# IntelLabs/bayesian-torch

Hardware: AMD Instinct MI355X
Metric: MC-samples/sec (Bayesian-ResNet18, 224^2, bs=64) (higher is better)
Workload: dtype bf16

## Files before the change

bayesian_torch_amd/_lib.py:

```python
import ctypes
import os

_HERE = os.path.dirname(os.path.abspath(__file__))
_LIB = None

KIND_REPARAM, KIND_FLIPOUT = 0, 1
ACT_F32, ACT_BF16 = 0, 1
PREC_F32, PREC_BF16, PREC_BF16X3 = 0, 1, 2
PREC_CODE = {"f32": 0, "bf16": 1, "bf16x3": 2}
FLAG_TRANSPOSED, FLAG_KL_ACCUM, FLAG_ROWFUSE, FLAG_OUT_F32, FLAG_OUT_BF16, FLAG_GATHER, FLAG_SWAP_SIGNS, FLAG_CONCURRENT = 1, 2, 4, 8, 16, 32, 64, 128
FLAG_REVERSE = 256
E_UNSUPPORTED = -3
STREAM_EPS_W, STREAM_EPS_B, STREAM_SIGN_IN, STREAM_SIGN_OUT = 0, 1, 2, 3
ABI_VERSION = 9
FLAG_LANES_SHIFT = 16
FLAG_LANES_MASK = 0xff << FLAG_LANES_SHIFT
SAMPLE_SKIP_MU = 1


class BtxError(RuntimeError):
    pass


class Geom(ctypes.Structure):
    _fields_ = [(n, ctypes.c_int32) for n in (
        "NB", "D", "H", "W", "C", "N", "KD", "KH", "KW", "sd", "sh", "sw", "pd", "ph", "pw",
        "dd", "dh", "dw", "od", "oh", "ow", "groups")]


class Rng(ctypes.Structure):
    _fields_ = [("seed", ctypes.c_uint64), ("sample_idx", ctypes.c_uint32), ("layer_id", ctypes.c_uint32),
                ("sample_idx_dev", ctypes.c_void_p)]


class BnFuse(ctypes.Structure):
    _fields_ = [("residual", ctypes.c_void_p), ("relu", ctypes.c_int32), ("mask", ctypes.c_void_p), ("dres", ctypes.c_void_p)]


class Epilogue(ctypes.Structure):
    _fields_ = [("scale", ctypes.c_void_p), ("shift", ctypes.c_void_p), ("residual", ctypes.c_void_p),
                ("relu", ctypes.c_int32), ("pool", ctypes.c_int32)]


class Lanes(ctypes.Structure):
    _fields_ = [("n", ctypes.c_int32), ("x_stride", ctypes.c_int64), ("out_stride", ctypes.c_int64),
                ("res_stride", ctypes.c_int64)]


class PlanInfo(ctypes.Structure):
    _fields_ = [(n, ctypes.c_int32) for n in ("family", "ksplits", "kper", "kgroups", "wide", "tall", "par_major", "pool_band",
                                              "nwg", "lanes")] + [("ws_bytes", ctypes.c_uint64)]


FAMILIES = ("gather", "regstage", "dma", "gemm8", "patch", "taps", "taps2", "stem", "stem_pool")


class Noise(ctypes.Structure):
    _fields_ = [("eps_w", ctypes.c_void_p), ("eps_b", ctypes.c_void_p),
                ("sign_in", ctypes.c_void_p), ("sign_out", ctypes.c_void_p), ("sampled_w", ctypes.c_void_p)]


class SampleItem(ctypes.Structure):
    _fields_ = [("geom", ctypes.POINTER(Geom)), ("mu_w", ctypes.c_void_p), ("rho_w", ctypes.c_void_p),
                ("out", ctypes.c_void_p), ("kind", ctypes.c_int32), ("layer_id", ctypes.c_uint32),
                ("src_KW", ctypes.c_int32), ("src_C", ctypes.c_int32)]


class LstmLayer(ctypes.Structure):
    _fields_ = [("mu_w", ctypes.c_void_p), ("rho_w", ctypes.c_void_p), ("mu_b", ctypes.c_void_p), ("rho_b", ctypes.c_void_p),
                ("layer_id", ctypes.c_uint32), ("sample_idx", ctypes.c_uint32), ("sample_idx_dev", ctypes.c_void_p)]


class LstmGrads(ctypes.Structure):
    _fields_ = [("dmu_w", ctypes.c_void_p), ("drho_w", ctypes.c_void_p), ("dmu_b", ctypes.c_void_p), ("drho_b", ctypes.c_void_p)]


class KlItem(ctypes.Structure):
    _fields_ = [("mu", ctypes.c_void_p), ("rho", ctypes.c_void_p), ("prior_mu_t", ctypes.c_void_p),
                ("prior_sigma_t", ctypes.c_void_p), ("dmu", ctypes.c_void_p), ("drho", ctypes.c_void_p),
                ("prior_mu", ctypes.c_float), ("prior_sigma", ctypes.c_float), ("n", ctypes.c_size_t)]


class Q8Chain(ctypes.Structure):
    _fields_ = [(n, ctypes.c_float) for n in ("s_sigma", "s_mu", "s_eps", "inv_s_eps", "s_d", "inv_s_d", "inv_s_w")] + \
               [("bias_div", ctypes.c_double)]


class Q8Add(ctypes.Structure):
    _fields_ = [(n, ctypes.c_float) for n in ("s_a", "pre_a", "s_b", "pre_b", "inv_s")] + \
               [("zero_point", ctypes.c_int32), ("relu", ctypes.c_int32)]


class Q8Delta(ctypes.Structure):
    _fields_ = [("inv_s_eps", ctypes.c_float), ("mult", ctypes.c_float), ("mean_bias", ctypes.c_int32), ("pert_bias", ctypes.c_int32),
# ... 247 lines not shown
```

bayesian_torch_amd/csrc/btx_contract_taps.h:

```cpp
#pragma once
#include <type_traits>
#include "btx_contract.h"
#include "btx_contract_dma.h"
#include "btx_epilogue.h"
#include "btx_mma.h"

namespace btx {

__device__ __forceinline__ void dma16s(__amdgpu_buffer_rsrc_t rsrc, uint32_t voff, uint32_t soff,
                                       unsigned char* lds_wave_base) {
  __builtin_amdgcn_raw_ptr_buffer_load_lds(rsrc, (__attribute__((address_space(3))) void*)lds_wave_base, 16, voff, soff,
                                           0, 0);
}

template <int N>
__device__ __forceinline__ void end_stage() {
  asm volatile("s_waitcnt vmcnt(%0)\n\ts_waitcnt lgkmcnt(0)\n\ts_barrier" ::"n"(N) : "memory");
}

template <int I, int N, class F>
__device__ __forceinline__ void static_for(F&& f) {
  if constexpr (I < N) {
    f(std::integral_constant<int, I>{});
    static_for<I + 1, N>(f);
// ... 264 lines not shown
            if constexpr (t == 0) write_signs(PAR ^ 1, cb0 + cbi + 1);
          }
        }
        DeltaFrag df;
        if constexpr (KG == 1) {
          load_delta<K2>(df, smem + PT_W_OFF + wslot * DW_STAGE, l31, h);
          constexpr int t1 = (t + 1) % T, c1 = (t + 1) / T;
          load_frag(nxt, PAR ^ c1, (t1 / KW) * row_step + (t1 % KW) * p.dw, (wslot + 1) & 3, mia_tag);
          if constexpr (FIRST && t == 0) stage_mma<PREC, K2, MI, MIA, true, KIND == 1>(cur, df, accm, accd, l31, h);
          else stage_mma<PREC, K2, MI, MIA, false, KIND == 1>(cur, df, accm, accd, l31, h);
          if (!last) end_stage<WOPS + KP>();
          else end_stage<(c3 == 0) ? WOPS : 0>();
        } else {
          load_delta<KIND>(df, smem + PT_W_OFF + wslot * DW_STAGE, l31, h);
          load_frag(cur, PAR, (t / KW) * row_step + (t % KW) * p.dw, wslot, mia_tag);
          __builtin_amdgcn_sched_barrier(0);
          asm volatile("s_barrier" ::: "memory");
          __builtin_amdgcn_sched_barrier(0);
          stage_mma<PREC, KIND, MI, MIA>(cur, df, accm, accd, l31, h);
          __builtin_amdgcn_sched_barrier(0);
          if (!last) {
            end_stage<2 * WOPS + KP + tp_pieces<T>(t - 1) + tp_pieces<T>(t - 2)>();
          } else {
            constexpr int a_ = (t + 3 < T) ? 1 : 0, b_ = (t == 0) ? 1 : ((t + 2 < T) ? 1 : 0);
            end_stage<WOPS * (a_ + b_)>();
          }
        }
        wslot = (wslot + 1) & 3;
      });
    };
    if (KG == 2 && kg == 1) asm volatile("s_barrier" ::: "memory");
    using P0 = std::integral_constant<int, 0>;
    using P1 = std::integral_constant<int, 1>;
    if constexpr (ZI) {
      if constexpr (MIA < MI) clear_acc(MIA);
      block(P0{}, std::true_type{}, 0, ncb == 1);
      int cbi = 1;
      for (; cbi + 2 <= ncb; cbi += 2) {
        block(P1{}, std::false_type{}, cbi, false);
        block(P0{}, std::false_type{}, cbi + 1, cbi + 2 == ncb);
      }
      if (cbi < ncb) block(P1{}, std::false_type{}, cbi, true);
    } else {
      int cbi = 0;
      for (; cbi + 2 <= ncb; cbi += 2) {
        block(P0{}, std::false_type{}, cbi, false);
        block(P1{}, std::false_type{}, cbi + 1, cbi + 2 == ncb);
      }
      if (cbi < ncb) block(P0{}, std::false_type{}, cbi, true);
    }
    if (KG == 2 && kg == 0) asm volatile("s_barrier" ::: "memory");
    };
    if (mi1_dead) kloop(std::integral_constant<int, 1>{});
    else kloop(std::integral_constant<int, 2>{});
  }

  {
    BTX_SECTION_PARAMS(pe, logical2);
    const int nimg = min(pe.pt_G, pe.NB - img0), nrow = min(pe.pt_R, pe.Ho - row0);
    const int nvalid = nimg * nrow * pe.Wo;
    const uint32_t m0 = (uint32_t)(img0 * pe.Ho + row0) * (uint32_t)pe.Wo;
    const PixTall pmt = {pe, row0, col0};
    if constexpr (KG == 1) {
      if constexpr (WIDE) {
        float* const ba0 = (float*)(smem + NW * PT_EP_WAVE);
        float* const ba1 = ba0 + 4 * BN;
        {
          const bool has_bias = (split == 0) && (pe.mu_b != nullptr);
          const bool has_aff = (pe.ksplits == 1) && ((pe.ep_scale != nullptr) || (pe.ep_shift != nullptr));
          if (has_bias || has_aff) {
            if (tid < 64) ep_fill_constants<0>(pe, rl, ba0, tid, 2 * ntile, group, has_bias, has_aff);
            else if (tid < 128) ep_fill_constants<0>(pe, rl, ba1, tid - 64, 2 * ntile + 1, group, has_bias, has_aff);
          }
          __syncthreads();
        }
        if (tall) {
          staged_epilogue_pm<0, NW, PixTall>(pe, rl, accm, accm, smem, tid, wave, lane, 2 * ntile, group, split, pmt, -1, true, ba0);
          staged_epilogue_pm<0, NW, PixTall>(pe, rl, accd, accd, smem, tid, wave, lane, 2 * ntile + 1, group, split, pmt, -1, true, ba1);
        } else {
          staged_epilogue<0, NW>(pe, rl, accm, accm, smem, tid, wave, lane, 2 * ntile, group, split, m0, nvalid, -1, true, ba0);
          staged_epilogue<0, NW>(pe, rl, accd, accd, smem, tid, wave, lane, 2 * ntile + 1, group, split, m0, nvalid, -1, true, ba1);
        }
      } else
      if (tall) staged_epilogue_pm<KIND, NW, PixTall>(pe, rl, accm, accd, smem, tid, wave, lane, ntile, group, split, pmt);
      else staged_epilogue<KIND, NW>(pe, rl, accm, accd, smem, tid, wave, lane, ntile, group, split, m0, nvalid);
    } else {
      float* ba_lds = (float*)(smem_all + 131072);
      const bool to_partial = pe.ksplits > 1;
      const bool has_bias = (split == 0) && (pe.mu_b != nullptr);
      const bool has_aff = !to_partial && ((pe.ep_scale != nullptr) || (pe.ep_shift != nullptr));
      if (kg == 1) {
#pragma unroll
        for (int mi = 0; mi < MI; ++mi)
#pragma unroll
          for (int ni = 0; ni < 2; ++ni)
#pragma unroll
            for (int c = 0; c < 4; ++c) {
              const int i = (mi * 2 + ni) * 4 + c;
              *(f32x4*)(smem_all + (i * 256 + tid) * 16) =
                  (f32x4){accm[mi][ni][4 * c], accm[mi][ni][4 * c + 1], accm[mi][ni][4 * c + 2], accm[mi][ni][4 * c + 3]};
              if constexpr (KIND == 1)
                *(f32x4*)(smem_all + ((16 + i) * 256 + tid) * 16) =
                    (f32x4){accd[mi][ni][4 * c], accd[mi][ni][4 * c + 1], accd[mi][ni][4 * c + 2], accd[mi][ni][4 * c + 3]};
            }
      } else if (has_bias || has_aff) {
        ep_fill_constants<KIND>(pe, rl, ba_lds, tid, ntile, group, has_bias, has_aff);
      }
      __syncthreads();
      if (kg == 0) {
#pragma unroll
        for (int mi = 0; mi < MI; ++mi)
#pragma unroll
          for (int ni = 0; ni < 2; ++ni)
#pragma unroll
            for (int c = 0; c < 4; ++c) {
              const int i = (mi * 2 + ni) * 4 + c;
              const f32x4 v = *(const f32x4*)(smem_all + (i * 256 + tid) * 16);
#pragma unroll
              for (int r = 0; r < 4; ++r) accm[mi][ni][4 * c + r] += v[r];
              if constexpr (KIND == 1) {
                const f32x4 w = *(const f32x4*)(smem_all + ((16 + i) * 256 + tid) * 16);
#pragma unroll
                for (int r = 0; r < 4; ++r) accd[mi][ni][4 * c + r] += w[r];
              }
            }
      }
      __syncthreads();
      if (kg == 0) {
        if (tall) staged_epilogue_pm<KIND, NW, PixTall>(pe, rl, accm, accd, smem_all, tid, wave, lane, ntile, group, split, pmt, -1,
                                                        true, ba_lds);
        else staged_epilogue<KIND, NW>(pe, rl, accm, accd, smem_all, tid, wave, lane, ntile, group, split, m0, nvalid, -1, true,
                                       ba_lds);
      }
    }
  }
}

}
```

bayesian_torch_amd/csrc/btx_epilogue.h:

```cpp
#pragma once
#include <type_traits>
#include "btx_contract.h"

namespace btx {

template <int I, int N, class F>
__device__ __forceinline__ void static_for_ep(F&& f) {
  if constexpr (I < N) {
    f(std::integral_constant<int, I>{});
    static_for_ep<I + 1, N>(f);
  }
}

struct EpRaw {
  float mu, rho, eps, sc, sh;
};
__device__ __forceinline__ EpRaw ep_load_constants(const ContractParams& p, int t, int ntile, int group, bool has_bias,
                                                   bool has_aff) {
  EpRaw r = {0.f, 0.f, 0.f, 1.f, 0.f};
  if (t < BN) {
    const int col = ntile * BN + t;
    const int gcol = group * p.Ng + (col < p.Ng ? col : 0);
    if (has_bias && col < p.Ng) {
      r.mu = p.mu_b[gcol];
// ... 20 lines not shown
    }
    ba_lds[t] = bm;
    ba_lds[BN + t] = bdl;
    ba_lds[2 * BN + t] = r.sc;
    ba_lds[3 * BN + t] = r.sh;
  }
}
template <int KIND>
__device__ __forceinline__ void ep_fill_constants(const ContractParams& p, const RngLive& rl, float* ba_lds, int t,
                                                  int ntile, int group, bool has_bias, bool has_aff) {
  const EpRaw r = ep_load_constants(p, t, ntile, group, has_bias, has_aff);
  ep_store_constants<KIND>(p, rl, r, ba_lds, t, ntile, group, has_bias);
}

struct PixContig {
  uint32_t m0;
  int nvalid;
  __device__ __forceinline__ uint32_t operator()(int pl, bool& ok) const { ok = pl < nvalid; return m0 + (uint32_t)pl; }
  __device__ __forceinline__ uint32_t first() const { return m0; }
  struct Walk {
    uint32_t g; int pl, nvalid;
    __device__ __forceinline__ uint32_t get(bool& ok) const { ok = pl < nvalid; return g; }
    __device__ __forceinline__ void step8() { g += 8u; pl += 8; }
  };
  __device__ __forceinline__ Walk walk(int pl) const { return Walk{m0 + (uint32_t)pl, pl, nvalid}; }
};
__device__ __forceinline__ uint32_t par_major_pixel(const ContractParams& p, uint32_t L) {
  uint32_t cls, q, t, b, nb, a;
  fdivmod(L, p.fd_par_Mqp, (uint32_t)p.par_Mqp, cls, q);
  fdivmod(q, p.fd_par_Wh, (uint32_t)p.par_Wh, t, b);
  fdivmod(t, p.fd_par_Hh, (uint32_t)p.par_Hh, nb, a);
  return (nb * (uint32_t)p.Ho + 2u * a + (cls >> 1)) * (uint32_t)p.Wo + 2u * b + (cls & 1u);
}
struct PixParity {
  const ContractParams& p;
  uint32_t m0;
  int nvalid;
  __device__ __forceinline__ uint32_t operator()(int pl, bool& ok) const {
    ok = pl < nvalid;
    return ok ? par_major_pixel(p, m0 + (uint32_t)pl) : 0u;
  }
  __device__ __forceinline__ uint32_t first() const { return 0u; }
  struct Walk {
    const ContractParams& p;
    uint32_t L; int pl, nvalid;
    __device__ __forceinline__ uint32_t get(bool& ok) const { ok = pl < nvalid; return ok ? par_major_pixel(p, L) : 0u; }
    __device__ __forceinline__ void step8() { L += 8u; pl += 8; }
  };
  __device__ __forceinline__ Walk walk(int pl) const { return Walk{p, m0 + (uint32_t)pl, pl, nvalid}; }
};
struct PixTall {
  const ContractParams& p;
  int row0, col0;
  __device__ __forceinline__ uint32_t operator()(int pl, bool& ok) const {
    uint32_t r, c, img, oh;
    fdivmod((uint32_t)pl, p.fd_Wt, (uint32_t)p.pt_Wt, r, c);
    fdivmod((uint32_t)row0 + r, p.fd_P, (uint32_t)p.pt_P, img, oh);
    const int ow = col0 + (int)c;
    ok = (int)r < p.pt_R && (int)oh < p.Ho && (int)img < p.NB && ow < p.Wo;
    return ok ? ((img * (uint32_t)p.Ho + oh) * (uint32_t)p.Wo + (uint32_t)ow) : 0u;
  }
  __device__ __forceinline__ uint32_t first() const { return 0u; }
  struct Walk {
    const ContractParams& p;
    int r, c, oh, img, col0;
    __device__ __forceinline__ uint32_t get(bool& ok) const {
      const int ow = col0 + c;
      ok = r < p.pt_R && oh < p.Ho && img < p.NB && ow < p.Wo;
      return ok ? (uint32_t)((img * p.Ho + oh) * p.Wo + ow) : 0u;
    }
    __device__ __forceinline__ void step8() {
      c += 8;
#pragma unroll
      for (int i = 0; i < 2; ++i)
        if (c >= p.pt_Wt) { c -= p.pt_Wt; ++r; if (++oh >= p.pt_P) { oh -= p.pt_P; ++img; } }
    }
  };
  __device__ __forceinline__ Walk walk(int pl) const {
    uint32_t r, c, img, oh;
    fdivmod((uint32_t)pl, p.fd_Wt, (uint32_t)p.pt_Wt, r, c);
    fdivmod((uint32_t)row0 + r, p.fd_P, (uint32_t)p.pt_P, img, oh);
    return Walk{p, (int)r, (int)c, (int)oh, (int)img, col0};
  }
};

struct EpNoHook {
  __device__ __forceinline__ void operator()() const {}
};
template <int KIND, int NW, class PM = PixContig, bool RES_PRE = false, class HOOK = EpNoHook>
__device__ __forceinline__ void staged_epilogue_pm(const ContractParams& p, const RngLive& rl, const f32x16 (&accm)[2][2],
                                                   const f32x16 (&accd)[2][2], unsigned char* smem, int tid, int wave,
                                                   int lane, int ntile, int group, int split, const PM& pm,
                                                   int pwave = -1, bool first = true,
                                                   float* ba_ext = nullptr, const HOOK& hook = HOOK{},
                                                   const uint32_t* wsh_ext = nullptr) {
  if (pwave < 0) pwave = wave;
  constexpr int EP_ROW = PT_EP_ROW;
  constexpr int EP_WAVE = PT_EP_WAVE;
  const int l31 = lane & 31, h = lane >> 5;
  const bool to_partial = p.ksplits > 1;
  const bool has_bias = (split == 0) && (p.mu_b != nullptr);
  const bool has_aff = !to_partial && ((p.ep_scale != nullptr) || (p.ep_shift != nullptr));
  const bool has_ba = has_bias || has_aff;
  float* ba_lds = ba_ext ? ba_ext : (float*)(smem + NW * EP_WAVE);
  if (has_ba && first && !ba_ext) {
    ep_fill_constants<KIND>(p, rl, ba_lds, tid, ntile, group, has_bias, has_aff);
    __syncthreads();
  }
  unsigned char* ep = smem + wave * EP_WAVE;

  constexpr bool BUFIO = RES_PRE && std::is_same<PM, PixContig>::value;
  u32x4 rpre[8];
  auto io_off = [&](int lane_) __attribute__((always_inline)) -> uint32_t {
    return ((pm.first() + (uint32_t)(pwave * 64 + (lane_ >> 3))) * (uint32_t)p.N + (uint32_t)(group * p.Ng + ntile * BN + (lane_ & 7) * 8)) * 2u;
  };
  const uint32_t io_step = 8u * (uint32_t)p.N * 2u, io_bytes = (uint32_t)p.M * (uint32_t)p.N * 2u;
  if constexpr (RES_PRE) {
    const bool all_vec = ((p.N & 7) == 0) && (((group * p.Ng) & 7) == 0) && (ntile * BN + BN <= p.Ng);
    if (all_vec && !to_partial && p.ep_res != nullptr && p.out_bf16 && p.ep_relu != 2) {
      if constexpr (BUFIO) {
        const __amdgpu_buffer_rsrc_t res_rsrc = __builtin_amdgcn_make_buffer_rsrc((void*)p.ep_res, 0, io_bytes, 0x00020000);
        const uint32_t io_voff = io_off(lane);
#pragma unroll
        for (int i = 0; i < 8; ++i) rpre[i] = __builtin_amdgcn_raw_buffer_load_b128(res_rsrc, io_voff, io_step * (uint32_t)i, 0);
      } else {
        const uint32_t cbase = (uint32_t)(group * p.Ng + ntile * BN + (lane & 7) * 8);
        auto wk = pm.walk(pwave * 64 + (lane >> 3));
#pragma unroll
        for (int i = 0; i < 8; ++i) {
          bool ok;
          const uint32_t gp = wk.get(ok);
          wk.step8();
          rpre[i] = *(const u32x4*)((const __bf16*)p.ep_res + (ok ? gp * (uint32_t)p.N + cbase : cbase + pm.first() * (uint32_t)p.N));
        }
      }
    }
  }

  hook();

  const bool fast = (ntile * BN + BN <= p.Ng) &&
                    (KIND == 0 || (!p.sign_out && (p.N & 31) == 0 && ((group * p.Ng) & 31) == 0));
  if (fast) {
    uint32_t wsh[2][2];
    uint32_t SB = 0x80000000u;
    asm volatile("" : "+s"(SB));
    if constexpr (KIND == 1) {
      if (wsh_ext) {
#pragma unroll
        for (int i = 0; i < 4; ++i) wsh[i >> 1][i & 1] = wsh_ext[i];
      } else {
#pragma unroll
        for (int mi = 0; mi < 2; ++mi) {
          bool pok;
          const uint32_t orow = pm(pwave * 64 + mi * 32 + l31, pok) * (uint32_t)p.N + (uint32_t)(group * p.Ng + ntile * BN);
#pragma unroll
          for (int ni = 0; ni < 2; ++ni)
            wsh[mi][ni] = btx_sign_word((orow + 32u * ni) >> 5, rl.kout_a, rl.kout_b) << (2 * h);
        }
      }
    }
    auto body = [&](auto bias_tag, auto aff_tag) __attribute__((always_inline)) {
      constexpr bool BIAS = decltype(bias_tag)::value, BA = decltype(aff_tag)::value;
      struct Cst { f32x4 bm, bd, sc, sh; };
      auto ldc = [&](int g, Cst& c) __attribute__((always_inline)) {
        const int cl = (g >> 2) * 32 + 8 * (g & 3) + 4 * h;
// ... 16 lines not shown
        const int cl = ni * 32 + 8 * q + 4 * h;
#pragma unroll
        for (int mi = 0; mi < 2; ++mi) {
          f32x4 v;
#pragma unroll
          for (int rr = 0; rr < 4; ++rr) {
            float val = accm[mi][ni][4 * q + rr];
            if constexpr (BIAS) val += cur.bm[rr];
            if constexpr (KIND == 1) {
              float dl = accd[mi][ni][4 * q + rr];
              if constexpr (BIAS) dl += cur.bd[rr];
              const int sft = 31 - (((rr & 1) ? 31 : 15) - 4 * q - (rr >> 1));
              val += u2f(__builtin_amdgcn_bitop3_b32(f2u(dl), wsh[mi][ni] << sft, SB, 0x78));
            }
            if constexpr (BA) val = __builtin_fmaf(val, cur.sc[rr], cur.sh[rr]);
            v[rr] = val;
          }
          *(f32x4*)(ep + (mi * 32 + l31) * EP_ROW + cl * 4) = v;
        }
      });
    };
    if (has_bias) body(std::true_type{}, std::true_type{});
    else if (has_ba) body(std::false_type{}, std::true_type{});
    else body(std::false_type{}, std::false_type{});
  } else {
#pragma unroll 1
    for (int mi = 0; mi < 2; ++mi) {
      bool pix_ok;
      const uint32_t gp_ = pm(pwave * 64 + mi * 32 + l31, pix_ok);
      const uint32_t orow = (pix_ok ? gp_ : pm.first()) * (uint32_t)p.N + (uint32_t)(group * p.Ng);
#pragma unroll
      for (int ni = 0; ni < 2; ++ni) {
#pragma unroll
        for (int q = 0; q < 4; ++q) {
          const int cl = ni * 32 + 8 * q + 4 * h;
          const int c0 = ntile * BN + cl;
          float v[4];
#pragma unroll
          for (int rr = 0; rr < 4; ++rr) {
            const int col = c0 + rr;
            float val = (mi == 0 ? accm[0][ni][4 * q + rr] : accm[1][ni][4 * q + rr]);
            if (has_ba) val += ba_lds[cl + rr];
            if constexpr (KIND == 1) {
              float dl = (mi == 0 ? accd[0][ni][4 * q + rr] : accd[1][ni][4 * q + rr]);
              if (has_ba) dl += ba_lds[BN + cl + rr];
              uint32_t flip = 0;
              if (col < p.Ng && pix_ok) {
                if (p.sign_out) {
                  flip = (p.sign_out[orow + col] < 0) ? 0x80000000u : 0u;
                } else {
                  const uint32_t io = orow + col;
                  const uint32_t w1 = btx_sign_word(io >> 5, rl.kout_a, rl.kout_b);
                  flip = (w1 << (31 - btx_sign_bitpos(io & 31u))) & 0x80000000u;
                }
              }
              val += u2f(f2u(dl) ^ flip);
            }
            if (has_ba) val = __builtin_fmaf(val, ba_lds[2 * BN + cl + rr], ba_lds[3 * BN + cl + rr]);
            v[rr] = val;
          }
          *(f32x4*)(ep + (mi * 32 + l31) * EP_ROW + cl * 4) = (f32x4){v[0], v[1], v[2], v[3]};
        }
      }
    }
  }
  asm volatile("s_waitcnt lgkmcnt(0)" ::: "memory");
  __builtin_amdgcn_sched_barrier(0);

  {
    const int cg = lane & 7;
    const int col0 = ntile * BN + cg * 8;
    const int nv = min(8, p.Ng - col0);
    const uint32_t cbase = (uint32_t)(group * p.Ng + col0);
    const bool all_vec = ((p.N & 7) == 0) && (((group * p.Ng) & 7) == 0) && (ntile * BN + BN <= p.Ng) && p.ep_relu != 2;
    const bool res = !to_partial && p.ep_res != nullptr, relu = !to_partial && p.ep_relu;
    const bool relu6 = relu && p.ep_relu == 2;
    auto fast = [&](auto outk_tag, auto res_tag, auto relu_tag) __attribute__((always_inline)) {
      constexpr int OUTK = decltype(outk_tag)::value;
      constexpr bool RES = decltype(res_tag)::value, RELU = decltype(relu_tag)::value;
      auto wk = pm.walk(pwave * 64 + (lane >> 3));
      int lane_s2 = lane;
      asm volatile("" : "+v"(lane_s2));
      const uint32_t io_voff = BUFIO ? io_off(lane_s2) : 0u;
      constexpr int NP = RES_PRE ? 8 : 4;
#pragma unroll
      for (int hf = 0; hf < 8 / NP; ++hf) {
        uint32_t idx[NP];
        bool pk[NP];
        u32x4 r0[NP], r1[NP];
#pragma unroll
        for (int i = 0; i < NP; ++i) {
          if constexpr (BUFIO && OUTK == 1) {
            pk[i] = true; idx[i] = 0;
            if constexpr (RES) r0[i] = rpre[hf * NP + i];
            continue;
          }
          const uint32_t gp = wk.get(pk[i]);
          wk.step8();
          idx[i] = gp * (uint32_t)p.N + cbase;
          if constexpr (RES) {
            const uint32_t li = pk[i] ? idx[i] : cbase + pm.first() * (uint32_t)p.N;
            if constexpr (OUTK == 1 && RES_PRE) r0[i] = rpre[hf * NP + i];
            else if constexpr (OUTK == 1) r0[i] = *(const u32x4*)((const __bf16*)p.ep_res + li);
            else { r0[i] = *(const u32x4*)((const float*)p.ep_res + li); r1[i] = *(const u32x4*)((const float*)p.ep_res + li + 4); }
          }
        }
        f32x4 lo[NP], hi[NP];
#pragma unroll
        for (int i = 0; i < NP; ++i) {
          const int pix = (hf * NP + i) * 8 + (lane >> 3);
          lo[i] = *(const f32x4*)(ep + pix * EP_ROW + cg * 32);
          hi[i] = *(const f32x4*)(ep + pix * EP_ROW + cg * 32 + 16);
        }
#pragma unroll
        for (int i = 0; i < NP; ++i) {
          float v[8] = {lo[i][0], lo[i][1], lo[i][2], lo[i][3], hi[i][0], hi[i][1], hi[i][2], hi[i][3]};
          if constexpr (RES) {
            if constexpr (OUTK == 1) {
#pragma unroll
              for (int j = 0; j < 4; ++j) { v[2 * j] += u2f(r0[i][j] << 16); v[2 * j + 1] += u2f(r0[i][j] & 0xffff0000u); }
            } else {
#pragma unroll
              for (int j = 0; j < 4; ++j) { v[j] += u2f(r0[i][j]); v[4 + j] += u2f(r1[i][j]); }
            }
          }
          if constexpr (RELU) {
#pragma unroll
            for (int j = 0; j < 8; ++j) v[j] = fmaxf(v[j], 0.f);
          }
          if constexpr (OUTK == 1 && !BUFIO) {
            const f32x4 x0 = {v[0], v[1], v[2], v[3]}, x1 = {v[4], v[5], v[6], v[7]};
            const u32x2 p0 = __builtin_bit_cast(u32x2, __builtin_convertvector(x0, bf16x4));
            const u32x2 p1 = __builtin_bit_cast(u32x2, __builtin_convertvector(x1, bf16x4));
            const __amdgpu_buffer_rsrc_t out_rsrc = __builtin_amdgcn_make_buffer_rsrc((void*)p.out, 0, io_bytes, 0x00020000);
            __builtin_amdgcn_raw_buffer_store_b128((u32x4){p0[0], p0[1], p1[0], p1[1]}, out_rsrc, pk[i] ? idx[i] * 2u : 0xfffffff0u, 0, 0);
          } else
          if (pk[i]) {
            if constexpr (OUTK == 0) {
              float* dst = p.partial + (size_t)split * p.M * p.N + idx[i];
              *(f32x4*)dst = (f32x4){v[0], v[1], v[2], v[3]};
              *(f32x4*)(dst + 4) = (f32x4){v[4], v[5], v[6], v[7]};
            } else if constexpr (OUTK == 1) {
              const f32x4 x0 = {v[0], v[1], v[2], v[3]}, x1 = {v[4], v[5], v[6], v[7]};
              const u32x2 p0 = __builtin_bit_cast(u32x2, __builtin_convertvector(x0, bf16x4));
              const u32x2 p1 = __builtin_bit_cast(u32x2, __builtin_convertvector(x1, bf16x4));
              if constexpr (BUFIO) {
                const __amdgpu_buffer_rsrc_t out_rsrc = __builtin_amdgcn_make_buffer_rsrc((void*)p.out, 0, io_bytes, 0x00020000);
                __builtin_amdgcn_raw_buffer_store_b128((u32x4){p0[0], p0[1], p1[0], p1[1]}, out_rsrc, io_voff,
                                                       io_step * (uint32_t)(hf * NP + i), 0);
              } else {
                *(u32x4*)((__bf16*)p.out + idx[i]) = (u32x4){p0[0], p0[1], p1[0], p1[1]};
              }
            } else {
              float* dst = (float*)p.out + idx[i];
              *(f32x4*)dst = (f32x4){v[0], v[1], v[2], v[3]};
              *(f32x4*)(dst + 4) = (f32x4){v[4], v[5], v[6], v[7]};
            }
          }
        }
      }
    };
    using T = std::true_type;
    using F = std::false_type;
    if (all_vec) {
      if (to_partial) fast(std::integral_constant<int, 0>{}, F{}, F{});
      else if (p.out_bf16) {
        if (res) { if (relu) fast(std::integral_constant<int, 1>{}, T{}, T{}); else fast(std::integral_constant<int, 1>{}, T{}, F{}); }
        else { if (relu) fast(std::integral_constant<int, 1>{}, F{}, T{}); else fast(std::integral_constant<int, 1>{}, F{}, F{}); }
      } else {
        if (res) { if (relu) fast(std::integral_constant<int, 2>{}, T{}, T{}); else fast(std::integral_constant<int, 2>{}, T{}, F{}); }
        else { if (relu) fast(std::integral_constant<int, 2>{}, F{}, T{}); else fast(std::integral_constant<int, 2>{}, F{}, F{}); }
      }
    } else {
      auto wk = pm.walk(pwave * 64 + (lane >> 3));
#pragma unroll 1
      for (int r8 = 0; r8 < 8; ++r8) {
        const int pix = r8 * 8 + (lane >> 3);
        bool pok;
        const uint32_t gp = wk.get(pok);
        wk.step8();
        if (pok && nv > 0) {
// ... 30 lines not shown
```

bayesian_torch_amd/csrc/btx_plan.cpp:

```cpp
#include <string.h>
#include "btx_plan.h"

namespace btx {

static inline long long plan_lanes(uint32_t flags) {
  const long long n = (flags >> BTX_FLAG_LANES_SHIFT) & 0xffu;
  return n > 1 ? n : 1;
}

static inline bool throughput_plan(uint32_t flags) { return (flags & BTX_FLAG_CONCURRENT) || plan_lanes(flags) > 1; }

static int split_k(long long base1, int units, int unit_cost, int max_split, bool full_splits, bool throughput, bool short_exit) {
  int ks = 1;
  long long best = -1;
  for (int c = 1; c <= max_split; ++c) {
    if (full_splits && units % c) continue;
    const int per = (units + c - 1) / c;
    const long long rounds = (base1 * c + SLOTS - 1) / SLOTS;
    const long long cost = rounds * (per * unit_cost + 4) + (c > 1 ? 1 : 0);
    if (best < 0 || cost < best) { best = cost; ks = c; }
    if (throughput && (base1 * c >= 64 || (short_exit && base1 * c >= 16 && per <= 16))) { ks = c; break; }
  }
  return ks;
}
// ... 28 lines not shown
static bool dma_shape_ok(const BtxGeom* g, int act_dtype, int prec, const Plan& pl) {
  if ((prec == BTX_PREC_BF16) != (act_dtype == BTX_ACT_BF16)) return false;
  const int bk = NG * (prec == BTX_PREC_BF16 ? 8 : 4);
  if (pl.Cg % bk) return false;
  const long long in_elems = (long long)g->NB * g->D * g->H * g->W * g->C;
  const long long esz = (act_dtype == BTX_ACT_BF16) ? 2 : 4;
  if (in_elems * esz >= 0xfff00000LL || (long long)pl.M * g->N >= 0x7fffffffLL ||
      (long long)g->N * pl.K * 4 >= 0xfff00000LL)
    return false;
  return true;
}

static double tall_tile(const BtxGeom* g, const Plan& pl, int tp, int ppcap, PatchPlan* pt) {
  const int halo_r = (g->KH - 1) * g->dh, halo_c = (g->KW - 1) * g->dw;
  if (g->ph > halo_r) return 0.0;
  const int P = (g->H + g->ph > pl.Ho) ? g->H + g->ph : pl.Ho;
  const long long rows_total = (long long)(g->NB - 1) * P + pl.Ho;
  double best = 0.0;
  for (int ncs = 1; ncs <= 8; ++ncs) {
    const int Wt = (pl.Wo + ncs - 1) / ncs;
    if (Wt > tp || Wt < 4 || (ncs > 1 && Wt < 8)) continue;
    int R = tp / Wt;
    if (R > rows_total) R = (int)rows_total;
    while (R >= 1 && (R + halo_r) * (Wt + halo_c) > ppcap) --R;
    if (R < 1) continue;
    const long long rtiles = (rows_total + R - 1) / R;
    const double eff = (double)pl.M / ((double)rtiles * ncs * tp);
    if (eff > best * 1.01) {
      best = eff;
      pt->tall = 1; pt->P = P; pt->Wt = Wt; pt->ncs = ncs;
      pt->G = 1; pt->R = R; pt->Rp = R + halo_r; pt->Wp = Wt + halo_c; pt->PP = pt->Rp * pt->Wp;
      pt->rtiles = (int)rtiles;
    }
  }
  return best;
}
static bool patch_tile(const BtxGeom* g, const Plan& pl, int tp, int ppcap, PatchPlan* pt) {
  const int Ho = pl.Ho, Wo = pl.Wo;
  const int Wp = Wo + (g->KW - 1) * g->dw, halo_r = (g->KH - 1) * g->dh;
  if (Wo > tp || Wp * (1 + halo_r) > ppcap) return false;
  int G = 1, R;
  if (Ho * Wo <= tp / 2 || (Ho * Wo <= tp && (Ho + halo_r) * Wp <= ppcap)) {
    R = Ho;
    const int Rp = R + halo_r;
    if (Rp * Wp > ppcap) return false;
    G = tp / (Ho * Wo);
    if (G > ppcap / (Rp * Wp)) G = ppcap / (Rp * Wp);
    if (G > g->NB) G = g->NB;
    if (G < 1) return false;
  } else {
    int rmax = tp / Wo;
    const int rfit = ppcap / Wp - halo_r;
    if (rfit < rmax) rmax = rfit;
    if (rmax > Ho) rmax = Ho;
    if (rmax < 1) return false;
    const int nrt = (Ho + rmax - 1) / rmax;
    R = (Ho + nrt - 1) / nrt;
    auto mfma_tiles = [&](int r) {
      long long n = 0;
      for (int row = 0; row < Ho; row += r) n += ((long long)((Ho - row < r) ? Ho - row : r) * Wo + 31) / 32;
      return n;
    };
    if (rmax > R && (Ho % rmax == 0 || 2 * (Ho % rmax) >= rmax) && mfma_tiles(rmax) < mfma_tiles(R)) R = rmax;
  }
  pt->G = G; pt->R = R; pt->Rp = R + halo_r; pt->Wp = Wp; pt->PP = G * pt->Rp * Wp;
  pt->rtiles = (Ho + R - 1) / R;
  return pt->PP <= ppcap && G * R * Wo <= tp;
}


static bool patch_base_ok(const BtxGeom* g, int act_dtype, int prec, uint32_t flags, Plan* pl, PatchPlan* pt) {
  if (flags & (BTX_FLAG_TRANSPOSED | BTX_FLAG_ROWFUSE)) return false;
  pt->wide = 0;
  if (make_plan(g, prec, flags, DBM, pl)) return false;
  if (!dma_shape_ok(g, act_dtype, prec, *pl)) return false;
  return g->D == 1 && g->KD == 1 && pl->Do == 1;
}
static bool patch_lds(PatchPlan* pt, int slots, int wd, int max_ni) {
  const int pieces = (pt->PP + 15) / 16;
  pt->NI = (pieces + pt->nw - 1) / pt->nw;
  if (pt->NI > max_ni) return false;
  pt->astage = pieces * 1024;
  int lds = slots * pt->astage + slots * (pt->astage / 16) + wd * 8192 + 1024;
  const int ep = pt->nw * PT_EP_WAVE + 1024;
  if (lds < ep) lds = ep;
  if (lds > (pt->nw == 4 ? 81920 : 163840)) return false;
  pt->lds = lds;
  pt->lds_g = (lds + 15) & ~15;
  return true;
}
static void wide_tile(const BtxGeom* g, int kind, int act_dtype, int prec, uint32_t flags, const Plan& pl, PatchPlan* pt) {
  if (kind == BTX_KIND_REPARAM && prec == BTX_PREC_BF16 && act_dtype == BTX_ACT_BF16 && (pl.Ng % 128) == 0 &&
      (long long)pl.mtiles * (pl.ntiles / 2) * g->groups * plan_lanes(flags) >= SLOTS) {
    pt->wide = 1;
    if (pt->lds < pt->nw * PT_EP_WAVE + 2048) {
      pt->lds = pt->nw * PT_EP_WAVE + 2048;
      pt->lds_g = (pt->lds + 15) & ~15;
    }
  }
}
static long long patch_base1(const BtxGeom* g, const Plan& pl, const PatchPlan& pt) {
  return (long long)pl.mtiles * (pt.wide ? pl.ntiles / 2 : pl.ntiles) * g->groups;
}
static bool patch_split_k(const BtxGeom* g, int prec, uint32_t flags, int T, Plan* pl, const PatchPlan& pt) {
  const int bk = NG * (prec == BTX_PREC_BF16 ? 8 : 4);
  const int units = pl->Cg / bk / pt.kg;
  const long long base1 = patch_base1(g, *pl, pt);
  const long long base1n = throughput_plan(flags) ? (long long)pl->mtiles * pl->ntiles * g->groups : base1;
  int max_ks = 1;
  while (max_ks < units && max_ks < 32 && (units + max_ks) / (max_ks + 1) * T >= 4) ++max_ks;
  const int ks = split_k(base1n, units, T, max_ks, pt.kg == 2, throughput_plan(flags), false);
  const int per = (units + ks - 1) / ks;
  pl->kper = per * pt.kg * bk;
  pl->ksplits = (units + per - 1) / per;
  const long long nwg = base1 * pl->ksplits;
  if (nwg > 0x7fffffffLL) return false;
  pl->nwg = (int)nwg;
  return true;
}

static bool make_patch_plan(const BtxGeom* g, int act_dtype, int prec, uint32_t flags, Plan* pl, PatchPlan* pt, int kind = -1) {
  if (!patch_base_ok(g, act_dtype, prec, flags, pl, pt) || g->sh != 1 || g->sw != 1) return false;
  const int T = g->KH * g->KW;
  if (T < 2 || T > 64) return false;
  pt->tall = 0; pt->P = 1; pt->Wt = 1; pt->ncs = 1;
  if (patch_tile(g, *pl, 256, 352, pt)) pt->nw = 4;
  else if (patch_tile(g, *pl, 512, 960, pt)) pt->nw = 8;
  else return false;
  if (pt->nw == 4 && g->KH == 3 && g->KW == 3) {
    const long long mt_old = (long long)((g->NB + pt->G - 1) / pt->G) * pt->rtiles;
    const double eff_old = (double)pl->M / ((double)mt_old * 256.0);
    PatchPlan tp = *pt;
    const double eff_tall = tall_tile(g, *pl, 256, 352, &tp);
    if (eff_tall > eff_old * TALL_MIN_GAIN) *pt = tp;
  }
  if (!patch_lds(pt, 2, PT_WD, PT_MAXNI)) return false;
  pl->mtiles = pt->tall ? pt->rtiles * pt->ncs : ((g->NB + pt->G - 1) / pt->G) * pt->rtiles;
  pt->taps = (pt->nw == 4 && pt->NI <= 6 && g->KH == 3 && g->KW == 3) ? 33 : 0;
  if (pt->taps == 33) wide_tile(g, kind, act_dtype, prec, flags, *pl, pt);
  const int ncb = pl->Cg / (NG * (prec == BTX_PREC_BF16 ? 8 : 4));
  pt->kg = (pt->taps && !throughput_plan(flags) && patch_base1(g, *pl, *pt) * plan_lanes(flags) <= 256 && ncb >= 2 && (ncb % 2) == 0 &&
            2 * pt->lds_g <= 163840) ? 2 : 1;
  if (!patch_split_k(g, prec, flags, T, pl, *pt)) return false;
  if (pt->kg == 2) pt->lds = 2 * pt->lds_g;
  return true;
}

static bool make_patch2_plan(const BtxGeom* g, int act_dtype, int prec, uint32_t flags, Plan* pl, PatchPlan* pt, int kind = -1) {
  if (!patch_base_ok(g, act_dtype, prec, flags, pl, pt)) return false;
  if (g->KH != 3 || g->KW != 3 || g->sh != 2 || g->sw != 2 || g->ph != 1 || g->pw != 1 || g->dh != 1 || g->dw != 1) return false;
  BtxGeom gp = *g;
  gp.KH = 2; gp.KW = 2;
  if (!patch_tile(&gp, *pl, 256, 272, pt)) return false;
  pt->nw = 4;
  pt->tall = 0; pt->P = 1; pt->Wt = 1; pt->ncs = 1;
  if (!patch_lds(pt, 3, 3, 5)) return false;
  pl->mtiles = ((g->NB + pt->G - 1) / pt->G) * pt->rtiles;
  wide_tile(g, kind, act_dtype, prec, flags, *pl, pt);
  pt->taps = 332;
  pt->kg = 1;
  return patch_split_k(g, prec, flags, 9, pl, *pt);
}

static bool make_stem_plan(const BtxGeom* g, int act_dtype, int prec, const Plan& pl, StemPlan* st) {
  if (g->D != 1 || g->KD != 1 || pl.Do != 1 || g->groups != 1) return false;
  const int esz = (act_dtype == BTX_ACT_BF16) ? 2 : 4;
  const int bk = NG * (prec == BTX_PREC_BF16 ? 8 : 4);
  if ((g->KW * g->C) % bk || pl.K % bk) return false;
  const long long rowB = (long long)g->W * g->C * esz;
  for (int nw = 4; nw <= 8; nw += 4) {
    const int tp = 64 * nw;
    if (pl.Wo > tp) continue;
    int R = tp / pl.Wo;
    if (R > pl.Ho) R = pl.Ho;
    const long long cap = (nw == 4 ? 81920 : 163840) - PT_WD * 8192;
    for (; R >= 1; --R) {
      const long long Rp = (long long)(R - 1) * g->sh + g->KH;
      const long long pb = Rp * rowB;
      const long long astage = (pb + 1023) / 1024 * 1024;
      const long long sbytes = ((pb / esz + 31) / 32 + 3) * 4;
      const long long sb16 = (sbytes + 15) / 16 * 16;
      if (astage + sb16 > cap) continue;
      long long lds = astage + sb16 + PT_WD * 8192;
      const long long ep = (long long)nw * PT_EP_WAVE + 1024;
      if (lds < ep) lds = ep;
      st->R = R; st->Rp = (int)Rp; st->rtiles = (pl.Ho + R - 1) / R; st->nw = nw; st->astage = (int)astage;
      st->sbytes = (int)sb16; st->lds = (int)lds; st->patch_bytes = (int)pb;
      const long long nwg = (long long)g->NB * st->rtiles * pl.ntiles;
      if (nwg > 0x7fffffffLL) return false;
      st->nwg = (int)nwg;
      return true;
    }
  }
  return false;
}

static bool make_stem_pool_plan(const BtxGeom* g, int act_dtype, int prec, const Plan& pl, StemPoolPlan* sp, int lanes = 1) {
  if (prec != BTX_PREC_BF16 || act_dtype != BTX_ACT_BF16) return false;
  if (g->D != 1 || g->KD != 1 || pl.Do != 1 || g->groups != 1) return false;
  const int bk = NG * 8;
  if ((g->KW * g->C) % bk || pl.K % bk || (g->N % 64)) return false;
  const int nstages = pl.K / bk;
  if (nstages < 1 || nstages > 7) return false;
  if (2 * pl.Wo > 256 || pl.Ho < 1) return false;
  const int Hq = (pl.Ho - 1) / 2 + 1, Wq = (pl.Wo - 1) / 2 + 1;
  const long long rowB = (long long)g->W * g->C * 2;
  const long long Rp = (long long)g->sh + g->KH;
  const long long pb = Rp * rowB;
  const long long astage = (pb + 1023) / 1024 * 1024;
  const long long sbytes = ((pb / 2 + 31) / 32 + 3) * 4;
  const long long sb16 = (sbytes + 127) / 128 * 128;
  const long long lds = (long long)nstages * 8192 + 3 * astage + 2 * sb16 + 3LL * pl.Wo * 128 + 1024 + 64;
  if (lds > 163840) return false;
  const long long units = (long long)g->NB * pl.ntiles;
  long long PB = ((long long)Hq * units * (lanes > 1 ? lanes : 1)) / 256;
  if (PB < 4) PB = 4;
  if (PB > Hq) PB = Hq;
  const int bands = (Hq + (int)PB - 1) / (int)PB;
  const long long nwg = units * bands;
  if (nwg > 0x7fffffffLL) return false;
  sp->PB = (int)PB; sp->bands = bands; sp->Rp = (int)Rp; sp->astage = (int)astage; sp->sbytes = (int)sb16;
  sp->lds = (int)lds; sp->patch_bytes = (int)pb; sp->nwg = (int)nwg; sp->Hq = Hq; sp->Wq = Wq;
  return true;
}

size_t patch_wt_bytes(const Plan& pl, const BtxGeom* g, int kind, int prec, size_t* one, int lanes) {
  const size_t arr = (size_t)g->groups * pl.ntiles * 64 * (size_t)pl.K * (prec == BTX_PREC_BF16 ? 2 : 4);
// ... 240 lines not shown
```

bayesian_torch_amd/csrc/btx_plan.h:

```cpp
#pragma once
#include <stddef.h>
#include <stdint.h>
#include "../../include/btx.h"

namespace btx {

constexpr int BM = 256;
constexpr int BN = 64;
constexpr int NG = 4;
constexpr int DBM = 512;

constexpr int PT_WD = 4;
constexpr int PT_EP_ROW = 272;
constexpr int PT_EP_WAVE = 64 * PT_EP_ROW;
constexpr int PT_MAXNI = 8;

constexpr long long SLOTS = 256;
constexpr double TALL_MIN_GAIN = 1.15;
constexpr int GEMM8_MIN_K = 128;
constexpr double WG_MAJOR_MIB = 3.0;

struct Plan {
  int Do, Ho, Wo, Cg, Ng, M, K, mtiles, ntiles, ksplits, kper, nwg;
};

struct PatchPlan {
  int G, R, Rp, Wp, PP, NI, rtiles, nw, astage, lds;
  int taps, kg, lds_g;
  int wide;
  int tall, P, Wt, ncs;
};

struct StemPlan {
  int R, Rp, rtiles, nw, astage, sbytes, lds, patch_bytes, nwg;
};

struct StemPoolPlan {
  int PB, bands, Rp, astage, sbytes, lds, patch_bytes, nwg, Hq, Wq;
};

struct FwdSel {
  int family;
  Plan pl;
  int par_major;
  int par_mqp, g8_pairs, out_bf16;
  StemPlan stp;
  StemPoolPlan spp;
  PatchPlan pt;
  size_t need, wt_off, wt_one, wt_all;
};
static inline bool uses_tiles(int family) { return family >= BTX_FAMILY_DMA; }

int select_fwd(int kind, const BtxGeom* g, int act_dtype, int prec, uint32_t flags, bool unaligned, const BtxNoise* noise,
               const BtxEpilogue* ep, FwdSel* s);

int make_plan(const BtxGeom* g, int prec, uint32_t flags, int bm, Plan* pl);
size_t plan_ws(const Plan& pl, const BtxGeom* g, int lanes = 1);
size_t patch_wt_bytes(const Plan& pl, const BtxGeom* g, int kind, int prec, size_t* one, int lanes = 1);

}
```

include/btx.h:

```cpp
#ifndef BTX_H_
#define BTX_H_

#include <stddef.h>
#include <stdint.h>

#ifdef __cplusplus
extern "C" {
#endif

#define BTX_ABI_VERSION 9

#define BTX_E_NULL        (-1)
#define BTX_E_SHAPE       (-2)
#define BTX_E_UNSUPPORTED (-3)
#define BTX_E_WORKSPACE   (-4)
#define BTX_E_DTYPE       (-5)
#define BTX_E_ALIGN       (-6)

#define BTX_KIND_REPARAM 0
#define BTX_KIND_FLIPOUT 1
#define BTX_ACT_F32  0
#define BTX_ACT_BF16 1
#define BTX_PREC_F32  0
#define BTX_PREC_BF16 1
#define BTX_PREC_BF16X3 2
#define BTX_FLAG_TRANSPOSED   1u
#define BTX_FLAG_KL_ACCUM     2u
#define BTX_FLAG_ROWFUSE      4u
#define BTX_FLAG_OUT_F32      8u
#define BTX_FLAG_OUT_BF16    16u
#define BTX_FLAG_SWAP_SIGNS  64u
#define BTX_FLAG_CONCURRENT 128u
#define BTX_FLAG_REVERSE    256u
#define BTX_FLAG_GATHER      32u

#define BTX_FLAG_LANES_SHIFT 16
#define BTX_FLAG_LANES_MASK  (0xffu << BTX_FLAG_LANES_SHIFT)
#define BTX_FLAG_LANES(n)    (((uint32_t)(n) & 0xffu) << BTX_FLAG_LANES_SHIFT)

#define BTX_STREAM_EPS_W    0u
#define BTX_STREAM_EPS_B    1u
#define BTX_STREAM_SIGN_IN  2u
#define BTX_STREAM_SIGN_OUT 3u

typedef struct BtxGeom {
  int32_t NB, D, H, W, C;
  int32_t N;
  int32_t KD, KH, KW;
  int32_t sd, sh, sw;
  int32_t pd, ph, pw;
  int32_t dd, dh, dw;
  int32_t od, oh, ow;
  int32_t groups;
} BtxGeom;

typedef struct BtxRng {
  uint64_t seed;
  uint32_t sample_idx;
  uint32_t layer_id;
  const uint32_t* sample_idx_dev;
} BtxRng;

typedef struct BtxNoise {
  const float*  eps_w;
  const float*  eps_b;
  const int8_t* sign_in;
  const int8_t* sign_out;
  const void*   sampled_w;
} BtxNoise;

int         btx_abi_version(void);
const char* btx_strerror(int code);

size_t btx_kl_workspace_bytes(size_t n);
int btx_kl_gauss(const float* mu, const float* rho, size_t n,
                 const float* prior_mu_t, const float* prior_sigma_t,
                 float prior_mu, float prior_sigma,
                 float* kl_out, uint32_t flags, void* ws, size_t ws_bytes, void* stream);

typedef struct BtxKlItem {
  const float* mu;
  const float* rho;
  const float* prior_mu_t;
  const float* prior_sigma_t;
  float*       dmu;
  float*       drho;
  float        prior_mu, prior_sigma;
  size_t       n;
} BtxKlItem;
size_t btx_kl_model_workspace_bytes(int n_items);
int btx_kl_gauss_model(const BtxKlItem* items_host, int n_items, float* kl_out, void* ws, size_t ws_bytes, void* stream);
int btx_kl_gauss_model_bwd(const BtxKlItem* items_host, int n_items, const float* grad_out, void* stream);

size_t btx_contract_workspace_bytes(const BtxGeom* g, int kind, int act_dtype, int prec, uint32_t flags);
int btx_contract_fwd(int kind, const BtxGeom* g,
                     const void* x, const float* mu_w, const float* rho_w,
                     const float* mu_b, const float* rho_b,
                     void* out,
                     const BtxRng* rng, const BtxNoise* noise ,
                     int act_dtype, int prec, uint32_t flags,
                     void* ws, size_t ws_bytes, void* stream);

typedef struct BtxEpilogue {
  const float* scale;
  const float* shift;
  const void*  residual;
  int32_t      relu;
  int32_t      pool;
} BtxEpilogue;
int btx_contract_pool_shape(const BtxGeom* g, int act_dtype, int prec, uint32_t flags, int32_t* Hq, int32_t* Wq);
int btx_contract_fwd_ex(int kind, const BtxGeom* g,
                        const void* x, const float* mu_w, const float* rho_w,
                        const float* mu_b, const float* rho_b,
                        void* out,
                        const BtxRng* rng, const BtxNoise* noise ,
                        int act_dtype, int prec, uint32_t flags,
                        void* ws, size_t ws_bytes, void* stream,
// ... 282 lines not shown
```

Baseline: 1938.

## Pick tall vs plain patch tiles by wave-round cost; precompute tall epilogue pixel table

In throughput mode, the planner now chooses between tall strip tiles and plain patch tiles by estimating how many 512-slot workgroup rounds each needs, weighted by a per-tile cost factor. New flags let callers force either layout. For tall tiles, the epilogue builds a per-thread LDS table of output pixel offsets once, instead of walking with fast-divmod per element. This adds 1 KB of LDS to the epilogue footprint and an extra LDS round trip.

Result: faster. 1958 (median of 6 runs) (+1.0%).

```diff
diff --git a/bayesian_torch_amd/_lib.py b/bayesian_torch_amd/_lib.py
--- a/bayesian_torch_amd/_lib.py
+++ b/bayesian_torch_amd/_lib.py
@@ -10,6 +10,7 @@
 PREC_CODE = {"f32": 0, "bf16": 1, "bf16x3": 2}
 FLAG_TRANSPOSED, FLAG_KL_ACCUM, FLAG_ROWFUSE, FLAG_OUT_F32, FLAG_OUT_BF16, FLAG_GATHER, FLAG_SWAP_SIGNS, FLAG_CONCURRENT = 1, 2, 4, 8, 16, 32, 64, 128
 FLAG_REVERSE = 256
+FLAG_TILES_PLAIN, FLAG_TILES_TALL = 512, 1024
 E_UNSUPPORTED = -3
 STREAM_EPS_W, STREAM_EPS_B, STREAM_SIGN_IN, STREAM_SIGN_OUT = 0, 1, 2, 3
 ABI_VERSION = 9
diff --git a/bayesian_torch_amd/csrc/btx_contract_taps.h b/bayesian_torch_amd/csrc/btx_contract_taps.h
--- a/bayesian_torch_amd/csrc/btx_contract_taps.h
+++ b/bayesian_torch_amd/csrc/btx_contract_taps.h
@@ -370,8 +370,15 @@
           staged_epilogue<0, NW>(pe, rl, accd, accd, smem, tid, wave, lane, 2 * ntile + 1, group, split, m0, nvalid, -1, true, ba1);
         }
       } else
-      if (tall) staged_epilogue_pm<KIND, NW, PixTall>(pe, rl, accm, accd, smem, tid, wave, lane, ntile, group, split, pmt);
-      else staged_epilogue<KIND, NW>(pe, rl, accm, accd, smem, tid, wave, lane, ntile, group, split, m0, nvalid);
+      if (tall) {
+        uint32_t* const otab = (uint32_t*)(smem + NW * PT_EP_WAVE + 1024);
+        bool ook;
+        const uint32_t ogp = pmt(tid, ook);
+        otab[tid] = ook ? ogp : PixTab::NONE;
+        asm volatile("s_waitcnt lgkmcnt(0)" ::: "memory");
+        const PixTab pmx = {otab};
+        staged_epilogue_pm<KIND, NW, PixTab>(pe, rl, accm, accd, smem, tid, wave, lane, ntile, group, split, pmx);
+      } else staged_epilogue<KIND, NW>(pe, rl, accm, accd, smem, tid, wave, lane, ntile, group, split, m0, nvalid);
     } else {
       float* ba_lds = (float*)(smem_all + 131072);
       const bool to_partial = pe.ksplits > 1;
diff --git a/bayesian_torch_amd/csrc/btx_epilogue.h b/bayesian_torch_amd/csrc/btx_epilogue.h
--- a/bayesian_torch_amd/csrc/btx_epilogue.h
+++ b/bayesian_torch_amd/csrc/btx_epilogue.h
@@ -126,6 +126,26 @@
     fdivmod((uint32_t)row0 + r, p.fd_P, (uint32_t)p.pt_P, img, oh);
     return Walk{p, (int)r, (int)c, (int)oh, (int)img, col0};
   }
+};
+struct PixTab {
+  static constexpr uint32_t NONE = 0xffffffffu;
+  const uint32_t* tab;
+  __device__ __forceinline__ uint32_t operator()(int pl, bool& ok) const {
+    const uint32_t e = tab[pl];
+    ok = e != NONE;
+    return ok ? e : 0u;
+  }
+  __device__ __forceinline__ uint32_t first() const { return 0u; }
+  struct Walk {
+    const uint32_t* t;
+    __device__ __forceinline__ uint32_t get(bool& ok) const {
+      const uint32_t e = *t;
+      ok = e != NONE;
+      return ok ? e : 0u;
+    }
+    __device__ __forceinline__ void step8() { t += 8; }
+  };
+  __device__ __forceinline__ Walk walk(int pl) const { return Walk{tab + pl}; }
 };
 
 struct EpNoHook {
@@ -308,6 +328,13 @@
       int lane_s2 = lane;
       asm volatile("" : "+v"(lane_s2));
       const uint32_t io_voff = BUFIO ? io_off(lane_s2) : 0u;
+      constexpr bool TAB = std::is_same<PM, PixTab>::value;
+      uint32_t tab_gp[8];
+      bool tab_ok[8];
+      if constexpr (TAB) {
+#pragma unroll
+        for (int i = 0; i < 8; ++i) { tab_gp[i] = wk.get(tab_ok[i]); wk.step8(); }
+      }
       constexpr int NP = RES_PRE ? 8 : 4;
 #pragma unroll
       for (int hf = 0; hf < 8 / NP; ++hf) {
@@ -321,8 +348,9 @@
             if constexpr (RES) r0[i] = rpre[hf * NP + i];
             continue;
           }
-          const uint32_t gp = wk.get(pk[i]);
-          wk.step8();
+          uint32_t gp;
+          if constexpr (TAB) { gp = tab_gp[hf * NP + i]; pk[i] = tab_ok[hf * NP + i]; }
+          else { gp = wk.get(pk[i]); wk.step8(); }
           idx[i] = gp * (uint32_t)p.N + cbase;
           if constexpr (RES) {
             const uint32_t li = pk[i] ? idx[i] : cbase + pm.first() * (uint32_t)p.N;
diff --git a/bayesian_torch_amd/csrc/btx_plan.cpp b/bayesian_torch_amd/csrc/btx_plan.cpp
--- a/bayesian_torch_amd/csrc/btx_plan.cpp
+++ b/bayesian_torch_amd/csrc/btx_plan.cpp
@@ -134,7 +134,7 @@
   if (pt->NI > max_ni) return false;
   pt->astage = pieces * 1024;
   int lds = slots * pt->astage + slots * (pt->astage / 16) + wd * 8192 + 1024;
-  const int ep = pt->nw * PT_EP_WAVE + 1024;
+  const int ep = pt->nw * PT_EP_WAVE + 1024 + PT_EP_PIX;
   if (lds < ep) lds = ep;
   if (lds > (pt->nw == 4 ? 81920 : 163840)) return false;
   pt->lds = lds;
@@ -154,11 +154,11 @@
 static long long patch_base1(const BtxGeom* g, const Plan& pl, const PatchPlan& pt) {
   return (long long)pl.mtiles * (pt.wide ? pl.ntiles / 2 : pl.ntiles) * g->groups;
 }
-static bool patch_split_k(const BtxGeom* g, int prec, uint32_t flags, int T, Plan* pl, const PatchPlan& pt) {
+static bool patch_split_k(const BtxGeom* g, int prec, uint32_t flags, int T, Plan* pl, const PatchPlan& pt, int mtiles_k = 0) {
   const int bk = NG * (prec == BTX_PREC_BF16 ? 8 : 4);
   const int units = pl->Cg / bk / pt.kg;
   const long long base1 = patch_base1(g, *pl, pt);
-  const long long base1n = throughput_plan(flags) ? (long long)pl->mtiles * pl->ntiles * g->groups : base1;
+  const long long base1n = throughput_plan(flags) ? (long long)(mtiles_k ? mtiles_k : pl->mtiles) * pl->ntiles * g->groups : base1;
   int max_ks = 1;
   while (max_ks < units && max_ks < 32 && (units + max_ks) / (max_ks + 1) * T >= 4) ++max_ks;
   const int ks = split_k(base1n, units, T, max_ks, pt.kg == 2, throughput_plan(flags), false);
@@ -179,22 +179,44 @@
   if (patch_tile(g, *pl, 256, 352, pt)) pt->nw = 4;
   else if (patch_tile(g, *pl, 512, 960, pt)) pt->nw = 8;
   else return false;
+  const PatchPlan plain = *pt;
+  PatchPlan strip = *pt;
+  bool has_tall = false, tall0 = false;
+  auto grid_mtiles = [&](const PatchPlan& f) { return f.tall ? f.rtiles * f.ncs : ((g->NB + f.G - 1) / f.G) * f.rtiles; };
   if (pt->nw == 4 && g->KH == 3 && g->KW == 3) {
-    const long long mt_old = (long long)((g->NB + pt->G - 1) / pt->G) * pt->rtiles;
-    const double eff_old = (double)pl->M / ((double)mt_old * 256.0);
-    PatchPlan tp = *pt;
-    const double eff_tall = tall_tile(g, *pl, 256, 352, &tp);
-    if (eff_tall > eff_old * TALL_MIN_GAIN) *pt = tp;
-  }
-  if (!patch_lds(pt, 2, PT_WD, PT_MAXNI)) return false;
-  pl->mtiles = pt->tall ? pt->rtiles * pt->ncs : ((g->NB + pt->G - 1) / pt->G) * pt->rtiles;
-  pt->taps = (pt->nw == 4 && pt->NI <= 6 && g->KH == 3 && g->KW == 3) ? 33 : 0;
-  if (pt->taps == 33) wide_tile(g, kind, act_dtype, prec, flags, *pl, pt);
-  const int ncb = pl->Cg / (NG * (prec == BTX_PREC_BF16 ? 8 : 4));
-  pt->kg = (pt->taps && !throughput_plan(flags) && patch_base1(g, *pl, *pt) * plan_lanes(flags) <= 256 && ncb >= 2 && (ncb % 2) == 0 &&
-            2 * pt->lds_g <= 163840) ? 2 : 1;
-  if (!patch_split_k(g, prec, flags, T, pl, *pt)) return false;
-  if (pt->kg == 2) pt->lds = 2 * pt->lds_g;
+    const double eff_old = (double)pl->M / ((double)grid_mtiles(plain) * 256.0);
+    const double eff_tall = tall_tile(g, *pl, 256, 352, &strip);
+    has_tall = eff_tall > 0.0;
+    tall0 = eff_tall > eff_old * TALL_MIN_GAIN;
+  }
+  auto lay_out = [&](const PatchPlan& f, int mtiles_k) {
+    *pt = f;
+    if (!patch_lds(pt, 2, PT_WD, PT_MAXNI)) return false;
+    pl->mtiles = grid_mtiles(f);
+    pt->taps = (pt->nw == 4 && pt->NI <= 6 && g->KH == 3 && g->KW == 3) ? 33 : 0;
+    if (pt->taps == 33) wide_tile(g, kind, act_dtype, prec, flags, *pl, pt);
+    const int ncb = pl->Cg / (NG * (prec == BTX_PREC_BF16 ? 8 : 4));
+    pt->kg = (pt->taps && !throughput_plan(flags) && patch_base1(g, *pl, *pt) * plan_lanes(flags) <= 256 && ncb >= 2 && (ncb % 2) == 0 &&
+              2 * pt->lds_g <= 163840) ? 2 : 1;
+    if (!patch_split_k(g, prec, flags, T, pl, *pt, mtiles_k)) return false;
+    if (pt->kg == 2) pt->lds = 2 * pt->lds_g;
+    return true;
+  };
+  const int mtiles0 = grid_mtiles(tall0 ? strip : plain);
+  if (!lay_out(tall0 ? strip : plain, mtiles0)) return false;
+  if (has_tall && pt->taps == 33 && throughput_plan(flags)) {
+    bool tall = tall0;
+    if (flags & BTX_FLAG_TILES_PLAIN) tall = false;
+    else if (flags & BTX_FLAG_TILES_TALL) tall = true;
+    else {
+      const long long per_m = (long long)pl->ntiles * g->groups * pl->ksplits * plan_lanes(flags);
+      const long long wg_plain = grid_mtiles(plain) * per_m, wg_tall = grid_mtiles(strip) * per_m;
+      if (wg_plain > ROUND_SLOTS)
+        tall = (double)((wg_tall + ROUND_SLOTS - 1) / ROUND_SLOTS) * TALL_TILE_COST <
+               (double)((wg_plain + ROUND_SLOTS - 1) / ROUND_SLOTS) * PLAIN_TILE_COST;
+    }
+    if (tall != tall0) return lay_out(tall ? strip : plain, mtiles0);
+  }
   return true;
 }
 
diff --git a/bayesian_torch_amd/csrc/btx_plan.h b/bayesian_torch_amd/csrc/btx_plan.h
--- a/bayesian_torch_amd/csrc/btx_plan.h
+++ b/bayesian_torch_amd/csrc/btx_plan.h
@@ -13,10 +13,13 @@
 constexpr int PT_WD = 4;
 constexpr int PT_EP_ROW = 272;
 constexpr int PT_EP_WAVE = 64 * PT_EP_ROW;
+constexpr int PT_EP_PIX = 1024;
 constexpr int PT_MAXNI = 8;
 
 constexpr long long SLOTS = 256;
 constexpr double TALL_MIN_GAIN = 1.15;
+constexpr long long ROUND_SLOTS = 512;
+constexpr double PLAIN_TILE_COST = 1.0, TALL_TILE_COST = 1.065;
 constexpr int GEMM8_MIN_K = 128;
 constexpr double WG_MAJOR_MIB = 3.0;
 
diff --git a/include/btx.h b/include/btx.h
--- a/include/btx.h
+++ b/include/btx.h
@@ -33,6 +33,8 @@
 #define BTX_FLAG_CONCURRENT 128u
 #define BTX_FLAG_REVERSE    256u
 #define BTX_FLAG_GATHER      32u
+#define BTX_FLAG_TILES_PLAIN 512u
+#define BTX_FLAG_TILES_TALL 1024u
 
 #define BTX_FLAG_LANES_SHIFT 16
 #define BTX_FLAG_LANES_MASK  (0xffu << BTX_FLAG_LANES_SHIFT)
```
